# google/ffn

Hardware: NVIDIA H100
Metric: fov_steps_per_sec (higher is better)
Workload: dtype f16

## Files before the change

### ffn_b200/_lib.py

```python

from __future__ import annotations

import ctypes as C
import os

import numpy as np

HERE = os.path.dirname(os.path.abspath(__file__))
LIB_PATH = os.path.join(HERE, 'libffn_b200.so')

COMPUTE_FP16_TC = 0
COMPUTE_FP32 = 1
COMPUTE_FP16X2_TC = 2
IMAGE_U8 = 0
IMAGE_F32 = 1
ARRAY_SEED = 0
ARRAY_SEGMENTATION = 1
ARRAY_QPROB = 2
ARRAY_IMAGE = 3
MASK_MOVEMENT = 0
MASK_SEED = 1
SEED_POLICY_KINDS = {'peaks_2d': 0, 'fill_empty': 1, 'max_peaks': 2}

EXPORTS = [
    'ffn_last_error', 'ffn_engine_create', 'ffn_engine_destroy', 'ffn_engine_set_compute_mode', 'ffn_engine_set_chains', 'ffn_engine_set_grid',
    'ffn_engine_info', 'ffn_engine_profile', 'ffn_engine_trace', 'ffn_predict', 'ffn_canvas_create', 'ffn_canvas_destroy',
    'ffn_canvas_set_mask', 'ffn_canvas_segment_at', 'ffn_canvas_segment_all',
    'ffn_canvas_update_at', 'ffn_canvas_init_seed', 'ffn_canvas_read', 'ffn_canvas_write',
    'ffn_canvas_policy_state_size', 'ffn_canvas_policy_state_get', 'ffn_canvas_policy_state_set',
    'ffn_canvas_set_resume', 'ffn_canvas_trace', 'ffn_canvas_seed_peaks', 'ffn_canvas_seed_policy', 'ffn_canvas_set_max_id', 'ffn_canvas_get_counters', 'ffn_canvas_spec_stats', 'ffn_canvas_device_ptr',
    'ffn_canvas_add_id_offset', 'ffn_decision_points', 'ffn_reseg_eval', 'ffn_selftest_wgmma',
]


class ModelDesc(C.Structure):
  _fields_ = [('fov_zyx', C.c_int32 * 3), ('deltas_zyx', C.c_int32 * 3), ('depth', C.c_int32),
              ('features', C.c_int32)]


class Options(C.Structure):
  _fields_ = [('init_activation', C.c_float), ('pad_value', C.c_float),
# ... 71 lines not shown
  lib = C.CDLL(LIB_PATH)
  p = C.c_void_p
  i32p = C.POINTER(C.c_int32)
  lib.ffn_last_error.restype = C.c_char_p
  lib.ffn_last_error.argtypes = []
  lib.ffn_engine_create.argtypes = [C.c_int, C.POINTER(ModelDesc), C.POINTER(C.c_void_p),
                                    C.POINTER(C.c_void_p), C.c_int, C.POINTER(p)]
  lib.ffn_engine_destroy.argtypes = [p]
  lib.ffn_engine_destroy.restype = None
  lib.ffn_engine_set_compute_mode.argtypes = [p, C.c_int]
  lib.ffn_engine_set_grid.argtypes = [p, C.c_int]
  lib.ffn_engine_set_chains.argtypes = [p, C.c_int]
  lib.ffn_engine_info.argtypes = [p, C.POINTER(C.c_int64)]
  lib.ffn_engine_profile.argtypes = [p, C.POINTER(C.c_int64), C.c_int]
  lib.ffn_engine_trace.argtypes = [p, C.POINTER(C.c_int64), C.c_int64, C.c_int]
  lib.ffn_predict.argtypes = [p, p, p, C.c_int, p]
  lib.ffn_canvas_create.argtypes = [p, p, C.c_int, i32p, C.c_float, C.c_float, C.POINTER(Options),
                                    C.c_int, C.POINTER(p)]
  lib.ffn_canvas_destroy.argtypes = [p]
  lib.ffn_canvas_destroy.restype = None
  lib.ffn_canvas_set_mask.argtypes = [p, C.c_int, p]
  lib.ffn_canvas_segment_at.argtypes = [p, i32p, C.c_int, C.c_int64, C.POINTER(SegStats)]
  lib.ffn_canvas_segment_all.argtypes = [p, p, C.c_int64, p, C.c_int64, C.POINTER(C.c_int64), p,
                                         C.c_int64, C.POINTER(C.c_int64), C.POINTER(Counters)]
  lib.ffn_canvas_update_at.argtypes = [p, i32p, p]
  lib.ffn_canvas_init_seed.argtypes = [p, i32p]
  lib.ffn_canvas_read.argtypes = [p, C.c_int, i32p, i32p, p]
  lib.ffn_canvas_write.argtypes = [p, C.c_int, i32p, i32p, p]
  lib.ffn_canvas_policy_state_size.argtypes = [p, C.POINTER(C.c_int64), C.POINTER(C.c_int64)]
  lib.ffn_canvas_policy_state_get.argtypes = [p, p, p, i32p]
# ... 32 lines not shown
```

### ffn_b200/csrc/device_types.cuh

```cuda
#pragma once

#include <cuda.h>
#include <cuda_fp16.h>
#include <cuda_runtime.h>
#include <stdint.h>

#include "../../include/ffn_b200.h"

namespace ffn {

constexpr int kThreads = 320;
constexpr int kLoadWarp = 8;
constexpr int kSigWarp = 9;
constexpr int kActStages = 3;
constexpr int kTileM = 128;
constexpr int kTileOut = 126;
constexpr int kStackN = 96;
constexpr int kFeat = 32;
constexpr int kAccRegs = 64 * kStackN / 128;
constexpr int kMaxConv = 32;
constexpr int kMaxChains = 4;
constexpr int kBufsPerChain = 6;
constexpr int kMaxBufs = kMaxChains * kBufsPerChain;
constexpr int kSplitShift = 10;
// ... 13 lines not shown
  int rows_alloc;
  int V;
  float inv_pp, inv_xp;
};

struct Weights {
  const __half* w16;
  const __half* w16x2;
  const float* w32;
  const float* bias;
  const float* w_lom;
  float b_lom;
};

constexpr int kTraceEvents = 8, kTraceTiles = 2048, kTraceCta = 1;

constexpr unsigned kRowValid = 1, kRowX0 = 2, kRowXLast = 4;

struct Workspace {
  const uint8_t* row_flags;
  __half* act0_l;
  __half* act_l[2];
  float4* act0_f;
  float4* act_f[2];
  float4* res;
  unsigned* bar;
  int* abort_flag;
  long long* prof;
};

struct CanvasDev {
  const void* image;
  int image_is_u8;
  float mean, stddev;
  int* seg;
// ... 141 lines not shown
  Sched* sched;
  Ctl* ctl;
  unsigned* round_flag;
  CUtensorMap tmap[kMaxChains][3];
  int use_tmap;
  float* snap;
  Job job;
  int compute_mode;
};

constexpr int kStateSlot = 352;
constexpr int kOffMisc = 160;
constexpr int kMiscAbort = 7, kMiscDisco = 8, kMiscScratch = 16;
constexpr int kOffRound = kOffMisc + (kMiscScratch + 32 * kMaxChains) * 4;
constexpr int kOffProf = kOffRound + 2 * kMaxChains * 8 * 4;
constexpr int kOffXchg = (kOffProf + 16 * 8 + 15) / 16 * 16;
constexpr int kXchgBytes = 2 * 8 * 2 * 4 * 8 * 4;
constexpr int kBarsAreaBytes = kOffXchg + kXchgBytes;

struct SmemLayout {
  int wbuf;
  int act;
  int bias;
  int bars;
  int total;
};

__host__ __device__ inline SmemLayout smem_layout(const Geom& g) {
  SmemLayout s;
  s.wbuf = 0;
  s.act = 2 * 27 * 4 * 512;
// ... 10 lines not shown
  int x = 1;
  bool valid = false;
  if (m >= 1 && m <= kTileOut && r >= 0 && r < g.nr) {
    const int rem = r % g.pp, y = rem / g.xp;
    x = rem % g.xp;
    valid = y < g.fy;
  }
  return (valid ? kRowValid : 0u) | (x == 0 ? kRowX0 : 0u) | (x == g.fx - 1 ? kRowXLast : 0u);
}

inline uint8_t row_flags_byte(const Geom& g, int tile, int warp, int gq) {
  const int m0 = warp * 16 + gq;
  return (uint8_t)(row_flags_of(g, tile, m0) | row_flags_of(g, tile, m0 + 8) << 4);
}

__host__ __device__ inline size_t w16_layer_offset_halfs(int layer) {
  return layer == 0 ? 0 : (size_t)27 * 2 * 256 + (size_t)(layer - 1) * 27 * 4 * 256;
}
__host__ __device__ inline size_t w32_layer_offset_floats(int layer) {
  return layer == 0 ? 0 : (size_t)27 * 4 * 32 + (size_t)(layer - 1) * 27 * 32 * 32;
}

}
```

### ffn_b200/csrc/engine.cu

```cuda
#include <algorithm>
#include <cmath>
#include <cstdio>
#include <cstdlib>
#include <cstring>
#include <memory>
#include <string>
#include <vector>

#include "device_types.cuh"
#define FFN_KNS plain
#define FFN_PROFILE 0
#include "flood_kernel.cuh"
#undef FFN_KNS
#undef FFN_PROFILE
#define FFN_KNS profiled
#define FFN_PROFILE 1
#include "flood_kernel.cuh"
#undef FFN_KNS
#undef FFN_PROFILE
#include "seed_kernels.cuh"
#include "decision_kernels.cuh"
#include "reseg_kernels.cuh"
#include "selftest.cuh"

// ... 181 lines not shown
  p.round_flag = e->d_round_flag;
  p.snap = c ? c->d_snap : nullptr;
  std::memcpy(p.tmap, e->tmap, sizeof(p.tmap));
  p.use_tmap = e->use_tmap;
  p.job = job;
  {
    const char* env = std::getenv("FFN_B200_WATCHDOG_S");
    const long long secs = env ? std::atoll(env) : 60;
    p.job.watchdog_ns = (secs > 0 ? secs : 60) * 1000000000ll;
  }
  p.compute_mode = e->compute_mode;
  CUDA_OK(cudaMemsetAsync(e->ws.bar, 0, sizeof(unsigned), cudaStreamPerThread));
  CUDA_OK(cudaMemsetAsync(e->ws.abort_flag, 0, sizeof(int), cudaStreamPerThread));
  CUDA_OK(cudaMemsetAsync(e->d_ctl, 0, sizeof(Ctl), cudaStreamPerThread));
  CUDA_OK(cudaMemsetAsync(e->d_round_flag, 0, sizeof(unsigned), cudaStreamPerThread));
  for (int k = 0; k < kMaxChains; ++k) CUDA_OK(cudaMemsetAsync(e->cws[k].bar, 0, sizeof(unsigned), cudaStreamPerThread));
  void* args[] = {&p};
  CUDA_OK(cudaEventRecord(e->ev0, cudaStreamPerThread));
  CUDA_OK(cudaLaunchCooperativeKernel(flood_kernel(e), dim3(e->grid), dim3(kThreads), args, (size_t)e->smem_bytes,
                                      cudaStreamPerThread));
  CUDA_OK(cudaEventRecord(e->ev1, cudaStreamPerThread));
  CUDA_OK(cudaStreamSynchronize(cudaStreamPerThread));
  float ms = 0.f;
  CUDA_OK(cudaEventElapsedTime(&ms, e->ev0, e->ev1));
  e->last_kernel_seconds = ms * 1e-3;
  e->launches++;
  int abort_flag = 0;
  CUDA_OK(cudaMemcpy(&abort_flag, e->ws.abort_flag, sizeof(int), cudaMemcpyDeviceToHost));
  if (abort_flag != 0)
    return fail("device-side wait timed out (abort code " + std::to_string(abort_flag) +
// ... 216 lines not shown
  e->w.w_lom = d_wlom;
  e->w.b_lom = biases[g.nconv][0];
  e->owned = {d_w16, d_w16x2, d_w32, d_bias, d_wlom};

  Workspace& ws = e->ws;
  const size_t ra = (size_t)g.rows_alloc;
  if (dev_alloc(&ws.act0_l, 2 * ra * 8)) return 1;
  if (dev_alloc(&ws.act_l[0], 4 * ra * 8)) return 1;
  if (dev_alloc(&ws.act_l[1], 4 * ra * 8)) return 1;
  if (dev_alloc(&ws.act0_f, ra)) return 1;
  if (dev_alloc(&ws.act_f[0], 8 * ra)) return 1;
  if (dev_alloc(&ws.act_f[1], 8 * ra)) return 1;
  if (dev_alloc(&ws.res, 8 * ra)) return 1;
  if (dev_alloc(&ws.bar, 1)) return 1;
  if (dev_alloc(&ws.abort_flag, 1)) return 1;
  if (dev_alloc(&ws.prof, 32 + kTraceEvents * kTraceTiles)) return 1;
  for (void* p : std::vector<void*>{ws.act0_l, ws.act_l[0], ws.act_l[1], ws.act0_f, ws.act_f[0], ws.act_f[1], ws.res,
                                    ws.bar, ws.abort_flag, ws.prof})
    e->owned.push_back(p);
  {
    std::vector<uint8_t> flags((size_t)g.nt * 64);
    for (int t = 0; t < g.nt; ++t)
      for (int i = 0; i < 64; ++i) flags[(size_t)t * 64 + i] = row_flags_byte(g, t, i / 8, i % 8);
    uint8_t* d_flags = nullptr;
    if (dev_alloc(&d_flags, flags.size())) return 1;
    e->owned.push_back(d_flags);
    CUDA_OK(cudaMemcpy(d_flags, flags.data(), flags.size(), cudaMemcpyHostToDevice));
    ws.row_flags = d_flags;
  }
  for (int k = 0; k < kMaxChains; ++k) {
    ChainDev& cw = e->cws[k];
    if (dev_alloc(&cw.act0_h, 2 * ra * 8)) return 1;
    if (dev_alloc(&cw.act_h[0], 4 * ra * 8)) return 1;
    if (dev_alloc(&cw.act_h[1], 4 * ra * 8)) return 1;
    if (dev_alloc(&cw.seed_raw[0], (size_t)g.nt * kTileM)) return 1;
    if (dev_alloc(&cw.seed_raw[1], (size_t)g.nt * kTileM)) return 1;
    if (dev_alloc(&cw.logits, (size_t)g.nt * kTileM)) return 1;
    if (dev_alloc(&cw.count, 4)) return 1;
    if (dev_alloc(&cw.bar, 1)) return 1;
    if (dev_alloc(&cw.res, (size_t)g.nt * kTileM * kFeat)) return 1;
    for (void* p : std::vector<void*>{cw.act0_h, cw.act_h[0], cw.act_h[1], cw.seed_raw[0], cw.seed_raw[1], cw.logits,
                                      cw.count, cw.bar, cw.res})
      e->owned.push_back(p);
// ... 67 lines not shown
}

int ffn_engine_info(FfnEngine* e, int64_t info[8]) {
  if (!e || !info) return fail("null argument");
  info[0] = e->sm_count;
  info[1] = e->grid;
  info[2] = e->smem_bytes;
  info[3] = e->g.nt;
  info[4] = e->g.nr;
  info[5] = e->g.V;
  info[6] = e->launches;
  info[7] = (int64_t)(e->last_kernel_seconds * 1e9);
  return 0;
}

int ffn_engine_profile(FfnEngine* e, int64_t out[32], int reset) {
  if (!e) return fail("null argument");
  if (!out) {
    e->profiling = reset != 0;
    return 0;
  }
  if (set_device(e)) return 1;
  long long h[32];
  CUDA_OK(cudaMemcpy(h, e->ws.prof, sizeof(h), cudaMemcpyDeviceToHost));
  for (int i = 0; i < 32; ++i) out[i] = h[i];
  if (reset) CUDA_OK(cudaMemset(e->ws.prof, 0, sizeof(h)));
  return 0;
}

int ffn_engine_trace(FfnEngine* e, int64_t* out, int64_t n, int reset) {
  if (!e || !out || n < 0 || n > (int64_t)kTraceEvents * kTraceTiles) return fail("bad argument");
  if (set_device(e)) return 1;
  static_assert(sizeof(long long) == sizeof(int64_t), "trace element");
  CUDA_OK(cudaMemcpy(out, e->ws.prof + 32, (size_t)n * sizeof(int64_t), cudaMemcpyDeviceToHost));
  if (reset) CUDA_OK(cudaMemset(e->ws.prof + 32, 0, sizeof(long long) * kTraceEvents * kTraceTiles));
  return 0;
}

int ffn_predict(FfnEngine* e, const float* seed, const float* image, int batch, float* logits_out) {
  if (!e || !seed || !image || !logits_out || batch < 1) return fail("bad argument");
  if (set_device(e)) return 1;
  const size_t n = (size_t)batch * e->g.V;
  if (batch > e->predict_cap) {
    cudaFree(e->d_in_seed);
    cudaFree(e->d_in_image);
    cudaFree(e->d_out);
    e->d_in_seed = e->d_in_image = e->d_out = nullptr;
    if (dev_alloc(&e->d_in_seed, n, false)) return 1;
    if (dev_alloc(&e->d_in_image, n, false)) return 1;
    if (dev_alloc(&e->d_out, n, false)) return 1;
// ... 1079 lines not shown
```

### ffn_b200/csrc/flood_kernel.cuh

```cuda

#include <math_constants.h>

#include <utility>

#include "device_types.cuh"
#include "sm90.cuh"

namespace ffn {
namespace FFN_KNS {

struct Ctx {
  const KParams* p;
  int tid, warp, lane, cta, G;
  int t_begin, t_end;
  unsigned bar_target;
  unsigned ev0, ev1, ev2, ev3, ev4;
  unsigned round;
  unsigned long long t_start;
  unsigned char* smem;
  float* s_bias;
  uint64_t* mb_w;
  uint64_t* mb_full;
  uint64_t* mb_empty;
  uint64_t* mb_sig;
// ... 18 lines not shown
  return k == 0 ? c.ev0 : (k == 1 ? c.ev1 : (k == 2 ? c.ev2 : (k == 3 ? c.ev3 : c.ev4)));
}
__device__ __forceinline__ void ev_add(Ctx& c, int k, unsigned n) {
  if (k == 0) c.ev0 += n;
  else if (k == 1) c.ev1 += n;
  else if (k == 2) c.ev2 += n;
  else if (k == 3) c.ev3 += n;
  else c.ev4 += n;
}
__device__ __forceinline__ CanvasState* chain_state(const Ctx& c, int k) {
  return reinterpret_cast<CanvasState*>(reinterpret_cast<unsigned char*>(c.s_state) + k * kStateSlot);
}

__device__ __forceinline__ void chain_tiles(const Ctx& c, int k, int& tb, int& te) {
  const int nt = c.p->g.nt, base = nt / c.G, extra = nt % c.G;
  const int q = (c.cta + c.G - (k * extra) % c.G) % c.G;
  tb = q * base + min(q, extra);
  te = tb + base + (q < extra ? 1 : 0);
}

__device__ __forceinline__ bool aborted(const Ctx& c) {
  return sm90::ld_volatile_s32(c.p->ws.abort_flag) != 0;
}

#if FFN_PROFILE
__device__ __forceinline__ long long prof_now(const Ctx& c) { return c.prof ? clock64() : 0ll; }
__device__ __forceinline__ void prof_add(const Ctx& c, int slot, long long dt) {
  if (c.prof) c.prof[slot] += dt;
}
__device__ __forceinline__ void trace_ev(const Ctx& c, int ev, unsigned idx) {
  long long* trace = c.p->ws.prof;
  if (trace && c.cta == kTraceCta && idx < (unsigned)kTraceTiles) trace[32 + ev * kTraceTiles + idx] = clock64();
}
#else
__device__ __forceinline__ long long prof_now(const Ctx&) { return 0ll; }
__device__ __forceinline__ void prof_add(const Ctx&, int, long long) {}
__device__ __forceinline__ void trace_ev(const Ctx&, int, unsigned) {}
#endif

__device__ __forceinline__ void mbar_wait(const Ctx& c, uint64_t* bar, uint32_t parity) {
  unsigned spins = 0;
  long long t0 = 0;
  while (!sm90::mbar_try_wait(bar, parity)) {
    if ((++spins & 0x3FF) == 0) {
      if (aborted(c)) return;
      const long long now = clock64();
      if (t0 == 0) t0 = now;
// ... 397 lines not shown
  if (!(layer & 1)) return tc_epilogue<EPI_A, X2>(c, k, layer, tile, e, flags, d);
  if (layer == 1) return tc_epilogue<EPI_B_FIRST, X2>(c, k, layer, tile, e, flags, d);
  return tc_epilogue<EPI_B, X2>(c, k, layer, tile, e, flags, d);
}

__device__ __forceinline__ void publish_counts(Ctx& c, int k, int hit) {
  hit = __reduce_add_sync(0xffffffffu, hit);
  if (c.lane == 0 && hit) atomicAdd(&c.s_misc[k], hit);
  asm volatile("bar.sync 5, 256;" ::: "memory");
  if (c.tid == 0 && c.s_misc[k]) {
    const unsigned packed = (unsigned)c.s_misc[k];
    unsigned* cnt = c.p->ch[k].count + 2 * (c.round & 1u);
    if (packed & 0xffffu) atomicAdd(cnt, packed & 0xffffu);
    if (packed >> 16) atomicAdd(cnt + 1, packed >> 16);
  }
}

__device__ __forceinline__ void layers_pipelined(Ctx& c, unsigned mask) {
  const KParams& p = *c.p;
  const Geom& g = p.g;
  unsigned char* act_smem = c.smem + 2 * 27 * 4 * 512;
  const int seg_rows = kTileOut + 2 * g.halo;
  const int stage_bytes = 3 * 4 * seg_rows * 16;
  const int nconv = g.nconv;
  if (c.tid == 0) prof_add(c, 11, -prof_now(c));

  if (c.warp == kLoadWarp) {
    for (int layer = 0; layer < nconv; ++layer) {
      const int nch = layer == 0 ? 2 : 4;
      const unsigned n0 = c.load_cnt;
// ... 83 lines not shown
            tc_mma_issue<4>(d, a_lo, b_lo, seg_rows, g.xp, std::make_integer_sequence<int, 18>{});
          }
          const unsigned flags = tc_row_flags(c, tile);
          sm90::wgmma_wait_all();
          __syncwarp();
          if (c.lane == 0) sm90::mbar_arrive(&c.mb_empty[s]);
          if (c.tid == 0) prof_add(c, 3, prof_now(c) - t0);
          if (c.tid == 0) trace_ev(c, 4, c.epi_cnt);
          t0 = prof_now(c);
          hit += tc_epilogue_any<false>(c, k, layer, tile, e, flags, d);
          if (c.tid == 0) prof_add(c, 5, prof_now(c) - t0);
          if (c.tid == 0) trace_ev(c, 6, c.epi_cnt - 1u);
        }
        if (layer == nconv - 1) {
          publish_counts(c, k, hit);
        } else {
          chain_arrive_epi(c, k);
        }
      }
    }
  }
  bit_set(c, 8, true);
#pragma unroll
  for (int k = 0; k < kMaxChains; ++k)
    if ((mask >> k) & 1u) ev_add(c, k, (unsigned)nconv);
  if (c.tid == 0) prof_add(c, 11, prof_now(c));
}

__device__ __forceinline__ void tc_layer_x2(Ctx& c, int layer) {
  const KParams& p = *c.p;
// ... 120 lines not shown
  __syncthreads();
}

template <bool kSplit>
__device__ __forceinline__ void layers_blocking(Ctx& c) {
  const KParams& p = *c.p;
  grid_barrier(c);
  for (int layer = 0; layer < p.g.nconv; ++layer) {
    if constexpr (kSplit) {
      tc_layer_x2(c, layer);
    } else {
      f32_layer(c, layer);
    }
    if (layer + 1 < p.g.nconv) grid_barrier(c);
  }
}

__device__ __forceinline__ void tail_paste(Ctx& c, int k, int b, unsigned par, int pz, int py, int px, int batch_idx, bool disco) {
  const KParams& p = *c.p;
  const Geom& g = p.g;
  const ChainDev& ch = p.ch[k];
  const bool predict = p.job.mode == MODE_PREDICT;
  for (int r = c.t_begin * kTileOut + c.tid; r < c.t_end * kTileOut; r += kThreads) {
    int z, y, x;
    if (!row_to_zyx(g, r, z, y, x)) continue;
    const size_t fi = ((size_t)z * g.fy + y) * g.fx + x;
    if (predict) {
      p.job.out_logits[(size_t)batch_idx * g.V + fi] = __ldcg(ch.logits + r);
      continue;
    }
// ... 58 lines not shown
  CanvasState* st = L.st;
  if (st->q_tail >= p.cv.q_cap) {
    st->overflow |= 1;
    return;
  }
  const int t = st->q_tail++;
  trace_event(p, st, EV_PUSH, z, y, x);
  p.ob[L.b].q_score[t] = score;
  p.ob[L.b].q_pos[3 * t + 0] = z;
  p.ob[L.b].q_pos[3 * t + 1] = y;
  p.ob[L.b].q_pos[3 * t + 2] = x;
}

__device__ __forceinline__ int* policy_scratch(const Ctx& c, int k) { return c.s_misc + kMiscScratch + 32 * k; }

__device__ __forceinline__ void face_argmax(const Ctx& c, const LChain& L, int face) {
  const KParams& p = *c.p;
  const Geom& g = p.g;
  const ChainDev& ch = p.ch[L.k];
  int* scr = policy_scratch(c, L.k);
  float* s_score = reinterpret_cast<float*>(scr);
  int* s_rel = scr + 8;
  int* s_ok = scr + 26;
  const int cz = g.fz / 2, cy = g.fy / 2, cx = g.fx / 2;
  const int axis = face >> 1;
  const int dax = axis == 0 ? g.dz : (axis == 1 ? g.dy : g.dx);
  const int off = (face & 1) ? dax : -dax;
  const int d0 = axis == 0 ? g.dy : g.dz;
  const int d1 = axis == 2 ? g.dy : g.dx;
  const int n0 = 2 * d0 + 1, n1 = 2 * d1 + 1;
  const float* lgp = ch.logits;
  const float* odp = ch.seed_raw[L.par];
  int ok = 0;
  if (dax != 0) {
    float best = -CUDART_INF_F;
    int best_i = 0x7fffffff;
    constexpr int kPerLane = 10;
    for (int base = c.lane; base < n0 * n1; base += 32 * kPerLane) {
      float lg[kPerLane], od[kPerLane];
#pragma unroll
      for (int u = 0; u < kPerLane; ++u) {
        const int e = base + 32 * u;
        lg[u] = 0.f;
        od[u] = 0.f;
        if (e < n0 * n1) {
          const int i0 = e / n1, i1 = e - i0 * n1;
          const int z = axis == 0 ? cz + off : cz - g.dz + i0;
          const int y = axis == 0 ? cy - g.dy + i0 : (axis == 1 ? cy + off : cy - g.dy + i1);
          const int x = axis == 2 ? cx + off : cx - g.dx + i1;
          const int row = z * g.pp + y * g.xp + x;
          lg[u] = __ldcg(lgp + row);
          if (L.disco) od[u] = __ldcg(odp + row);
        }
      }
#pragma unroll
      for (int u = 0; u < kPerLane; ++u) {
        const int e = base + 32 * u;
        if (e < n0 * n1) {
          float v = lg[u];
          if (L.disco && od[u] < 0.f && v > od[u]) v = od[u];
          if (v > best || best_i == 0x7fffffff) {
            best = v;
            best_i = e;
          }
        }
      }
    }
#pragma unroll
    for (int s = 16; s > 0; s >>= 1) {
      const float ov = __shfl_xor_sync(0xffffffffu, best, s);
      const int oi = __shfl_xor_sync(0xffffffffu, best_i, s);
      if (oi != 0x7fffffff && (best_i == 0x7fffffff || ov > best || (ov == best && oi < best_i))) {
        best = ov;
        best_i = oi;
      }
    }
    if (c.lane == 0) {
      ok = (best >= p.cv.policy_th_f32) ? 1 : 0;
      const int i0 = best_i / n1, i1 = best_i - i0 * n1;
      const int r0 = i0 - n0 / 2, r1 = i1 - n1 / 2;
      s_score[face] = best;
      s_rel[3 * face + 0] = axis == 0 ? off : r0;
      s_rel[3 * face + 1] = axis == 0 ? r0 : (axis == 1 ? off : r1);
      s_rel[3 * face + 2] = axis == 2 ? off : r1;
    }
  }
  if (c.lane == 0) s_ok[face] = ok;
}

__device__ __forceinline__ void policy_finish(const Ctx& c, const LChain& L) {
  const KParams& p = *c.p;
  const ObjDev& ob = p.ob[L.b];
  CanvasState* st = L.st;
  int* scr = policy_scratch(c, L.k);
  const float* s_score = reinterpret_cast<const float*>(scr);
  const int* s_rel = scr + 8;
  const int* s_ok = scr + 26;
  const unsigned full = 0xffffffffu;
  const int f = c.lane;
  const bool mine = f < 6 && s_ok[f] != 0;
  const float sc = f < 6 ? s_score[f] : 0.f;
  const int rz = f < 6 ? s_rel[3 * f] : 0, ry = f < 6 ? s_rel[3 * f + 1] : 0, rx = f < 6 ? s_rel[3 * f + 2] : 0;
// ... 742 lines not shown
  if (c.tid == 0 && sm90::globaltimer_ns() - c.t_start > (unsigned long long)p.job.watchdog_ns) atomicExch(p.ws.abort_flag, 5);
  for (int i = c.tid; i < K * kStateWords; i += 256) {
    if (c.tid >= 256) break;
    const int k = i / kStateWords, w = i - k * kStateWords;
    const int b = __ldcg(&p.sched->active[k]);
    reinterpret_cast<unsigned long long*>(chain_state(c, k))[w] =
        __ldcg(reinterpret_cast<const unsigned long long*>(p.ob[b].st) + w);
  }
  if (c.tid >= 256)
    for (int i = c.tid - 256; i < kSchedWords; i += kThreads - 256)
      reinterpret_cast<unsigned long long*>(sc)[i] = __ldcg(reinterpret_cast<const unsigned long long*>(p.sched) + i);
  if (c.tid >= kThreads - kMaxChains) {
    const int k = c.tid - (kThreads - kMaxChains);
    if (k < K) c.s_misc[kMiscDisco + k] = (((stepped >> k) & 1u) && disco_active(p, k, par)) ? 1 : 0;
  }
  __syncthreads();
  const long long t_pol = prof_now(c);
  if (p.job.mode != MODE_UPDATE_AT) {
    for (int t = c.warp; t < K * 6; t += kThreads / 32) {
      const int k = t / 6, f = t - 6 * k;
      if (!((stepped >> k) & 1u)) continue;
      LChain L{k, sc->active[k], chain_state(c, k), par, c.s_misc[kMiscDisco + k] != 0};
      face_argmax(c, L, f);
    }
  }
  __syncthreads();
  if (c.warp < K && ((stepped >> c.warp) & 1u)) {
    LChain L{c.warp, sc->active[c.warp], chain_state(c, c.warp), par, c.s_misc[kMiscDisco + c.warp] != 0};
    if (L.st->phase == PH_AFTER_STEP) after_step(c, L);
  }
  if (c.tid == 0) prof_add(c, 12, prof_now(c) - t_pol);
  __syncthreads();
  if (c.warp == 0) {
    if (c.lane == 0) {
      sc->steps_executed += __popc(stepped);
    }
    __syncwarp();
    bool pause = false;
    if (p.job.step_budget > 0 && p.job.mode == MODE_SEGMENT) {
      const CanvasState* s0 = chain_state(c, 0);
      pause = s0->seg_all ? sc->steps_executed >= p.job.step_budget : s0->ctr.inference_calls >= p.job.step_budget;
    }
    int acts[kMaxChains];
    bool any = false;
#pragma unroll
    for (int k = 0; k < kMaxChains; ++k) {
      acts[k] = ACT_EXIT;
// ... 40 lines not shown
        if (!any) a = ACT_EXIT;
        else if (a == ACT_EXIT && k < K) a = ACT_IDLE;
        p.ctl->action[k] = k < K ? a : ACT_EXIT;
        if (k < K) {
          const CanvasState* s = chain_state(c, k);
          p.ctl->pos[k][0] = s->cur[0];
          p.ctl->pos[k][1] = s->cur[1];
          p.ctl->pos[k][2] = s->cur[2];
          p.ctl->buf[k] = sc->active[k];
        }
      }
    }
    __syncwarp();
  }
  __syncthreads();
  for (int i = c.tid; i < K * kStateWords; i += 256) {
    if (c.tid >= 256) break;
    const int k = i / kStateWords, w = i - k * kStateWords;
    reinterpret_cast<unsigned long long*>(p.ob[sc->active[k]].st)[w] = reinterpret_cast<const unsigned long long*>(chain_state(c, k))[w];
  }
  if (c.tid >= 256)
    for (int i = c.tid - 256; i < kSchedWords; i += kThreads - 256)
      reinterpret_cast<unsigned long long*>(p.sched)[i] = reinterpret_cast<const unsigned long long*>(sc)[i];
  __syncthreads();
  if (c.tid == 0) {
    sm90::red_release_add(p.round_flag, 1u);
    prof_add(c, 8, prof_now(c) - t_all);
  }
}

__device__ __forceinline__ void load3(const int* src, int (&dst)[3]) {
  dst[0] = __ldcg(src);
  dst[1] = __ldcg(src + 1);
  dst[2] = __ldcg(src + 2);
}

__device__ __forceinline__ void clear_dirty(Ctx& c, int b) {
  const KParams& p = *c.p;
  const CanvasState* st = p.ob[b].st;
  int dlo[3], dhi[3];
  load3(st->dirty_lo, dlo);
// ... 149 lines not shown
  c.mb_w = reinterpret_cast<uint64_t*>(smem_raw + L.bars);
  c.mb_full = c.mb_w + 2;
  c.mb_empty = c.mb_full + kActStages;
  c.mb_sig = c.mb_empty + kActStages;
  c.load_cnt = c.epi_cnt = 0;
  c.s_misc = reinterpret_cast<int*>(smem_raw + L.bars + kOffMisc);
  c.s_round = reinterpret_cast<int*>(smem_raw + L.bars + kOffRound);
  c.s_xchg = reinterpret_cast<float*>(smem_raw + L.bars + kOffXchg);
  c.s_state = reinterpret_cast<CanvasState*>(smem_raw + L.bars + kOffXchg);
  c.s_sched = reinterpret_cast<Sched*>(smem_raw + L.bars + kOffXchg + kMaxChains * kStateSlot);
  static_assert((2 + 2 * kActStages + kMaxChains) * 8 <= kOffMisc, "mbarrier area");
  static_assert(kMaxChains * kStateSlot + (int)sizeof(Sched) <= kXchgBytes, "leader working copies");
  c.prof = nullptr;
  if (FFN_PROFILE && p.ws.prof && (c.cta == 0 || c.cta == c.G - 1)) {
    c.prof = reinterpret_cast<long long*>(smem_raw + L.bars + kOffProf);
    if (c.tid < 16) c.prof[c.tid] = c.tid == 10 ? -clock64() : 0;
  }
#if FFN_PROFILE
  c.sig_cnt = 0;
#endif
  c.bits = 0;
  const bool tc = p.compute_mode != FFN_COMPUTE_FP32;
  const int K = p.nchains;

  for (int i = c.tid; i < p.g.nconv * 32; i += kThreads) c.s_bias[i] = p.w.bias[i];
  if (c.tid < 32) c.s_bias[p.g.nconv * 32 + c.tid] = p.w.w_lom[c.tid];
  if (c.tid == 0) c.s_bias[p.g.nconv * 32 + 32] = p.w.b_lom;
  if (c.tid < 2 * kMaxChains * 8) c.s_round[c.tid] = 0;
  if (tc) {
    if (c.tid == 0) {
      sm90::mbar_init(&c.mb_w[0], 1);
// ... 49 lines not shown
          const bool disco = disco_active(p, k, ppar);
          tail_paste(c, k, cur[4], ppar, cur[1], cur[2], cur[3], 0, disco);
          if (c.tid == 0) {
            prev[0] = 1 | (disco ? 2 : 0);
            prev[1] = cur[1];
            prev[2] = cur[2];
            prev[3] = cur[3];
            prev[4] = cur[4];
          }
        } else if (c.tid == 0) {
          prev[0] = 0;
        }
      }
      if (c.tid == 0) prof_add(c, 7, prof_now(c) - t_paste);
      if (c.tid == 0) {
        spin_until(c, p.round_flag, c.round + 1u, 4);
        c.s_misc[kMiscAbort] = sm90::ld_volatile_s32(p.ws.abort_flag);
      }
      __syncthreads();
      const int abort_now = c.s_misc[kMiscAbort];
      if (c.tid < K) {
        int* cur = c.s_round + 8 * c.tid;
        cur[0] = sm90::ld_volatile_s32(&p.ctl->action[c.tid]);
        cur[1] = sm90::ld_volatile_s32(&p.ctl->pos[c.tid][0]);
        cur[2] = sm90::ld_volatile_s32(&p.ctl->pos[c.tid][1]);
        cur[3] = sm90::ld_volatile_s32(&p.ctl->pos[c.tid][2]);
        cur[4] = sm90::ld_volatile_s32(&p.ctl->buf[c.tid]);
      }
      __syncthreads();
      if (abort_now != 0) break;
      bool all_exit = true;
// ... 17 lines not shown
          commit_write(c, b);
        }
      }
      if (c.tid == 0) prof_add(c, 6, prof_now(c) - t0);
      if (mask) {
        run_layers<kSplit>(c, mask);
        if (c.tid == 0) prof_add(c, 9, __popc(mask));
      }
      stepped = mask;
      ++c.round;
    }
  }

  if (c.tid == 0) prof_add(c, 10, prof_now(c));
  __syncthreads();
  if (c.prof && c.tid < 16) p.ws.prof[(c.cta == 0 ? 0 : 16) + c.tid] += c.prof[c.tid];
  if (tc && c.warp == 0 && bit_get(c, 8)) mbar_wait(c, &c.mb_w[0], bit_get(c, 0));
}

}

#ifndef FFN_MISC_KERNELS_DEFINED
#define FFN_MISC_KERNELS_DEFINED
__global__ void relabel_offset_kernel(int* seg, size_t n, int offset) {
  const size_t stride = (size_t)gridDim.x * blockDim.x;
  for (size_t i = (size_t)blockIdx.x * blockDim.x + threadIdx.x; i < n; i += stride) {
    const int v = seg[i];
    if (v > 0) seg[i] = v + offset;
  }
}

// ... 35 lines not shown
```

### ffn_b200/engine.py

```python

from __future__ import annotations

import ctypes as C
from typing import Optional, Sequence

import numpy as np
from scipy.special import logit

from . import _lib


def f32_logit(p: float) -> float:
  return float(np.float32(logit(float(np.float32(p)))))


def make_options(init_activation=0.95, pad_value=0.05, move_threshold=0.9, segment_threshold=0.6,
                 disco_seed_threshold=0.0, min_boundary_dist_zyx=(1, 1, 1), min_segment_size=1000,
                 policy_score_threshold: Optional[float] = None) -> _lib.Options:
  o = _lib.Options()
  o.init_activation = f32_logit(init_activation)
  o.pad_value = f32_logit(pad_value)
  o.move_threshold = f32_logit(move_threshold)
  o.segment_threshold = f32_logit(segment_threshold)
  o.disco_seed_threshold = float(np.float32(disco_seed_threshold))
# ... 58 lines not shown
  def set_chains(self, max_chains: int):
    _lib.check(self._lib.ffn_engine_set_chains(self._h, int(max_chains)))

  def set_compute_mode(self, mode: int):
    _lib.check(self._lib.ffn_engine_set_compute_mode(self._h, int(mode)))
    self.compute_mode = int(mode)

  def info(self) -> dict:
    buf = (C.c_int64 * 8)()
    _lib.check(self._lib.ffn_engine_info(self._h, buf))
    keys = ('sm_count', 'grid', 'smem_bytes', 'tiles', 'rows', 'fov_voxels', 'launches', 'last_kernel_ns')
    return dict(zip(keys, [int(v) for v in buf]))

  PROFILE_SLOTS = ('barrier_wait', 'act_tma_wait', 'weight_wait', 'mma', 'unused4', 'epi_body',
                   'stage', 'paste', 'leader', 'steps', 'kernel', 'conv_layers', 'leader_policy', 'leader_pops',
                   'chain_barrier_wait', 'unused')

  def enable_profiling(self, on: bool = True):
    _lib.check(self._lib.ffn_engine_profile(self._h, None, 1 if on else 0))

  def profile(self, reset: bool = True) -> dict:
    buf = (C.c_int64 * 32)()
    _lib.check(self._lib.ffn_engine_profile(self._h, buf, 1 if reset else 0))
    return {'cta0': dict(zip(self.PROFILE_SLOTS, [int(v) for v in buf[:16]])),
            'cta_last': dict(zip(self.PROFILE_SLOTS, [int(v) for v in buf[16:32]]))}

  def trace(self, reset: bool = True) -> np.ndarray:
    buf = np.zeros((8, 2048), dtype=np.int64)
    _lib.check(self._lib.ffn_engine_trace(self._h, buf.ctypes.data_as(C.POINTER(C.c_int64)), buf.size, 1 if reset else 0))
    return buf

  def predict(self, seed: np.ndarray, image: np.ndarray) -> np.ndarray:
    seed = np.ascontiguousarray(seed, dtype=np.float32)
    image = np.ascontiguousarray(image, dtype=np.float32)
    if seed.shape != image.shape:
      raise ValueError('seed and image shapes differ')
    single = seed.ndim == 3
    if seed.shape[-3:] != self.fov_zyx:
      raise ValueError('patch shape %r does not match the model FoV %r' % (seed.shape[-3:], self.fov_zyx))
    batch = 1 if single else seed.shape[0]
# ... 204 lines not shown
```

### include/ffn_b200.h

```cpp
#ifndef FFN_B200_H_
#define FFN_B200_H_

#include <stdint.h>

#ifdef __cplusplus
extern "C" {
#endif

typedef struct FfnEngine FfnEngine;
typedef struct FfnCanvas FfnCanvas;

enum {
  FFN_COMPUTE_FP16_TC = 0,
  FFN_COMPUTE_FP32 = 1,
  FFN_COMPUTE_FP16X2_TC = 2
};

enum { FFN_IMAGE_U8 = 0, FFN_IMAGE_F32 = 1 };

enum { FFN_ARRAY_SEED = 0, FFN_ARRAY_SEGMENTATION = 1, FFN_ARRAY_QPROB = 2, FFN_ARRAY_IMAGE = 3 };

enum { FFN_MASK_MOVEMENT = 0, FFN_MASK_SEED = 1 };

typedef struct {
// ... 54 lines not shown
  int64_t max_id;
  double device_seconds;
  int64_t kernel_launches;
} FfnCounters;

const char* ffn_last_error(void);

int ffn_engine_create(int device, const FfnModelDesc* model, const float* const* weights_dhwio,
                      const float* const* biases, int compute_mode, FfnEngine** out);
void ffn_engine_destroy(FfnEngine* engine);
int ffn_engine_set_compute_mode(FfnEngine* engine, int compute_mode);
int ffn_engine_set_chains(FfnEngine* engine, int max_chains);
int ffn_engine_set_grid(FfnEngine* engine, int num_ctas);
int ffn_engine_info(FfnEngine* engine, int64_t info[8]);

int ffn_engine_profile(FfnEngine* engine, int64_t out[32], int reset);
int ffn_engine_trace(FfnEngine* engine, int64_t* out, int64_t n, int reset);

int ffn_predict(FfnEngine* engine, const float* seed, const float* image, int batch,
                float* logits_out);

int ffn_canvas_create(FfnEngine* engine, const void* image, int image_dtype,
                      const int32_t shape_zyx[3], float image_mean, float image_stddev,
                      const FfnOptions* options, int keep_probability_maps, FfnCanvas** out);
void ffn_canvas_destroy(FfnCanvas* canvas);
int ffn_canvas_set_mask(FfnCanvas* canvas, int which, const uint8_t* mask);

int ffn_canvas_segment_at(FfnCanvas* canvas, const int32_t start_zyx[3], int reset,
                          int64_t max_steps, FfnSegStats* out);

int ffn_canvas_segment_all(FfnCanvas* canvas, const int32_t* seeds_zyx, int64_t n_seeds,
// ... 96 lines not shown
```

Baseline: 6353.

## Fuse face argmax into last conv layer epilogue via distributed atomic reduction

Moves the per-face argmax of the movement policy out of the single-CTA leader and into the last conv layer. Each CTA reduces the face voxels that fall in its own tiles, using a precomputed face table, and writes the result into global slots with packed 64-bit atomicMax keys. The leader then only unpacks six keys per chain instead of scanning face voxels serially. This is meant to shorten the serial leader phase between steps, at the cost of extra atomics and a table lookup in every CTA. The change also adds a spare-CTA offset to the chain tile assignment and widens the profiling slots.

```diff
diff --git a/ffn_b200/_lib.py b/ffn_b200/_lib.py
--- a/ffn_b200/_lib.py
+++ b/ffn_b200/_lib.py
@@ -24,7 +24,7 @@
 
 EXPORTS = [
     'ffn_last_error', 'ffn_engine_create', 'ffn_engine_destroy', 'ffn_engine_set_compute_mode', 'ffn_engine_set_chains', 'ffn_engine_set_grid',
-    'ffn_engine_info', 'ffn_engine_profile', 'ffn_engine_trace', 'ffn_predict', 'ffn_canvas_create', 'ffn_canvas_destroy',
+    'ffn_engine_info', 'ffn_engine_profile', 'ffn_engine_trace', 'ffn_face_table', 'ffn_predict', 'ffn_canvas_create', 'ffn_canvas_destroy',
     'ffn_canvas_set_mask', 'ffn_canvas_segment_at', 'ffn_canvas_segment_all',
     'ffn_canvas_update_at', 'ffn_canvas_init_seed', 'ffn_canvas_read', 'ffn_canvas_write',
     'ffn_canvas_policy_state_size', 'ffn_canvas_policy_state_get', 'ffn_canvas_policy_state_set',
@@ -126,6 +126,8 @@
   lib.ffn_engine_info.argtypes = [p, C.POINTER(C.c_int64)]
   lib.ffn_engine_profile.argtypes = [p, C.POINTER(C.c_int64), C.c_int]
   lib.ffn_engine_trace.argtypes = [p, C.POINTER(C.c_int64), C.c_int64, C.c_int]
+  lib.ffn_face_table.argtypes = [C.POINTER(ModelDesc), C.c_int64, C.POINTER(C.c_int32), C.POINTER(C.c_int64),
+                                 C.POINTER(C.c_int32), C.POINTER(C.c_int64)]
   lib.ffn_predict.argtypes = [p, p, p, C.c_int, p]
   lib.ffn_canvas_create.argtypes = [p, p, C.c_int, i32p, C.c_float, C.c_float, C.POINTER(Options),
                                     C.c_int, C.POINTER(p)]
diff --git a/ffn_b200/csrc/device_types.cuh b/ffn_b200/csrc/device_types.cuh
--- a/ffn_b200/csrc/device_types.cuh
+++ b/ffn_b200/csrc/device_types.cuh
@@ -4,6 +4,10 @@
 #include <cuda_fp16.h>
 #include <cuda_runtime.h>
 #include <stdint.h>
+#include <string.h>
+
+#include <algorithm>
+#include <vector>
 
 #include "../../include/ffn_b200.h"
 
@@ -51,11 +55,21 @@
 };
 
 constexpr int kTraceEvents = 8, kTraceTiles = 2048, kTraceCta = 1;
+constexpr int kProfSlots = 32;
 
 constexpr unsigned kRowValid = 1, kRowX0 = 2, kRowXLast = 4;
+
+struct alignas(8) FaceEntry {
+  int row;
+  int face_e;
+};
+constexpr int kFaceSlots = 12;
 
 struct Workspace {
   const uint8_t* row_flags;
+  const FaceEntry* face_tab;
+  const int* face_first;
+  unsigned long long* face_best;
   __half* act0_l;
   __half* act_l[2];
   float4* act0_f;
@@ -227,7 +241,7 @@
 constexpr int kMiscAbort = 7, kMiscDisco = 8, kMiscScratch = 16;
 constexpr int kOffRound = kOffMisc + (kMiscScratch + 32 * kMaxChains) * 4;
 constexpr int kOffProf = kOffRound + 2 * kMaxChains * 8 * 4;
-constexpr int kOffXchg = (kOffProf + 16 * 8 + 15) / 16 * 16;
+constexpr int kOffXchg = (kOffProf + kProfSlots * 8 + 15) / 16 * 16;
 constexpr int kXchgBytes = 2 * 8 * 2 * 4 * 8 * 4;
 constexpr int kBarsAreaBytes = kOffXchg + kXchgBytes;
 
@@ -268,6 +282,43 @@
   return (uint8_t)(row_flags_of(g, tile, m0) | row_flags_of(g, tile, m0 + 8) << 4);
 }
 
+inline void build_face_table(const Geom& g, std::vector<FaceEntry>& tab, std::vector<int>& first) {
+  const int c[3] = {g.fz / 2, g.fy / 2, g.fx / 2}, d[3] = {g.dz, g.dy, g.dx};
+  tab.clear();
+  for (int face = 0; face < 6; ++face) {
+    const int axis = face >> 1, a0 = axis == 0 ? 1 : 0, a1 = axis == 2 ? 1 : 2;
+    if (d[axis] == 0) continue;
+    const int n1 = 2 * d[a1] + 1;
+    for (int e = 0; e < (2 * d[a0] + 1) * n1; ++e) {
+      int zyx[3];
+      zyx[axis] = c[axis] + ((face & 1) ? d[axis] : -d[axis]);
+      zyx[a0] = c[a0] - d[a0] + e / n1;
+      zyx[a1] = c[a1] - d[a1] + e % n1;
+      tab.push_back({zyx[0] * g.pp + zyx[1] * g.xp + zyx[2], face << 24 | e});
+    }
+  }
+  std::stable_sort(tab.begin(), tab.end(), [](const FaceEntry& a, const FaceEntry& b) { return a.row < b.row; });
+  first.assign((size_t)g.nt + 1, 0);
+  for (int t = 0, i = 0; t <= g.nt; ++t) {
+    while (i < (int)tab.size() && tab[i].row < t * kTileOut) ++i;
+    first[t] = i;
+  }
+}
+
+__host__ __device__ inline unsigned long long face_key(float score, int e) {
+  if (score == 0.f) score = 0.f;
+  unsigned b;
+  memcpy(&b, &score, 4);
+  b ^= (b >> 31) ? 0xffffffffu : 0x80000000u;
+  return (unsigned long long)b << 32 | (0xffffffffu - (unsigned)e);
+}
+__host__ __device__ inline void face_key_unpack(unsigned long long key, float& score, int& e) {
+  unsigned b = (unsigned)(key >> 32);
+  b ^= (b >> 31) ? 0x80000000u : 0xffffffffu;
+  memcpy(&score, &b, 4);
+  e = (int)(0xffffffffu - (unsigned)key);
+}
+
 __host__ __device__ inline size_t w16_layer_offset_halfs(int layer) {
   return layer == 0 ? 0 : (size_t)27 * 2 * 256 + (size_t)(layer - 1) * 27 * 4 * 256;
 }
diff --git a/ffn_b200/csrc/engine.cu b/ffn_b200/csrc/engine.cu
--- a/ffn_b200/csrc/engine.cu
+++ b/ffn_b200/csrc/engine.cu
@@ -219,6 +219,7 @@
   CUDA_OK(cudaMemsetAsync(e->ws.abort_flag, 0, sizeof(int), cudaStreamPerThread));
   CUDA_OK(cudaMemsetAsync(e->d_ctl, 0, sizeof(Ctl), cudaStreamPerThread));
   CUDA_OK(cudaMemsetAsync(e->d_round_flag, 0, sizeof(unsigned), cudaStreamPerThread));
+  CUDA_OK(cudaMemsetAsync(e->ws.face_best, 0, sizeof(unsigned long long) * kMaxChains * kFaceSlots, cudaStreamPerThread));
   for (int k = 0; k < kMaxChains; ++k) CUDA_OK(cudaMemsetAsync(e->cws[k].bar, 0, sizeof(unsigned), cudaStreamPerThread));
   void* args[] = {&p};
   CUDA_OK(cudaEventRecord(e->ev0, cudaStreamPerThread));
@@ -465,7 +466,7 @@
   if (dev_alloc(&ws.res, 8 * ra)) return 1;
   if (dev_alloc(&ws.bar, 1)) return 1;
   if (dev_alloc(&ws.abort_flag, 1)) return 1;
-  if (dev_alloc(&ws.prof, 32 + kTraceEvents * kTraceTiles)) return 1;
+  if (dev_alloc(&ws.prof, 2 * kProfSlots + kTraceEvents * kTraceTiles)) return 1;
   for (void* p : std::vector<void*>{ws.act0_l, ws.act_l[0], ws.act_l[1], ws.act0_f, ws.act_f[0], ws.act_f[1], ws.res,
                                     ws.bar, ws.abort_flag, ws.prof})
     e->owned.push_back(p);
@@ -478,6 +479,21 @@
     e->owned.push_back(d_flags);
     CUDA_OK(cudaMemcpy(d_flags, flags.data(), flags.size(), cudaMemcpyHostToDevice));
     ws.row_flags = d_flags;
+  }
+  {
+    std::vector<FaceEntry> tab;
+    std::vector<int> first;
+    build_face_table(g, tab, first);
+    FaceEntry* d_tab = nullptr;
+    int* d_first = nullptr;
+    if (dev_alloc(&d_tab, std::max<size_t>(tab.size(), 1))) return 1;
+    if (dev_alloc(&d_first, first.size())) return 1;
+    if (dev_alloc(&ws.face_best, (size_t)kMaxChains * kFaceSlots)) return 1;
+    for (void* p : std::vector<void*>{d_tab, d_first, ws.face_best}) e->owned.push_back(p);
+    CUDA_OK(cudaMemcpy(d_tab, tab.data(), tab.size() * sizeof(FaceEntry), cudaMemcpyHostToDevice));
+    CUDA_OK(cudaMemcpy(d_first, first.data(), first.size() * sizeof(int), cudaMemcpyHostToDevice));
+    ws.face_tab = d_tab;
+    ws.face_first = d_first;
   }
   for (int k = 0; k < kMaxChains; ++k) {
     ChainDev& cw = e->cws[k];
@@ -575,17 +591,36 @@
   return 0;
 }
 
-int ffn_engine_profile(FfnEngine* e, int64_t out[32], int reset) {
+int ffn_engine_profile(FfnEngine* e, int64_t out[64], int reset) {
   if (!e) return fail("null argument");
   if (!out) {
     e->profiling = reset != 0;
     return 0;
   }
   if (set_device(e)) return 1;
-  long long h[32];
+  static_assert(2 * kProfSlots == 64, "ffn_engine_profile's out[64]");
+  long long h[2 * kProfSlots];
   CUDA_OK(cudaMemcpy(h, e->ws.prof, sizeof(h), cudaMemcpyDeviceToHost));
-  for (int i = 0; i < 32; ++i) out[i] = h[i];
+  for (int i = 0; i < 2 * kProfSlots; ++i) out[i] = h[i];
   if (reset) CUDA_OK(cudaMemset(e->ws.prof, 0, sizeof(h)));
+  return 0;
+}
+
+int ffn_face_table(const FfnModelDesc* model, int64_t cap, int32_t* entries, int64_t* n_entries, int32_t* tile_first,
+                   int64_t* n_tiles) {
+  if (!model || !n_entries || !n_tiles) return fail("null argument");
+  const Geom g = make_geom(*model);
+  std::vector<FaceEntry> tab;
+  std::vector<int> first;
+  build_face_table(g, tab, first);
+  *n_entries = (int64_t)tab.size();
+  *n_tiles = g.nt;
+  for (size_t i = 0; entries && i < tab.size() && (int64_t)i < cap; ++i) {
+    entries[3 * i] = tab[i].row;
+    entries[3 * i + 1] = tab[i].face_e >> 24;
+    entries[3 * i + 2] = tab[i].face_e & 0xffffff;
+  }
+  if (tile_first) std::copy(first.begin(), first.end(), tile_first);
   return 0;
 }
 
@@ -593,8 +628,8 @@
   if (!e || !out || n < 0 || n > (int64_t)kTraceEvents * kTraceTiles) return fail("bad argument");
   if (set_device(e)) return 1;
   static_assert(sizeof(long long) == sizeof(int64_t), "trace element");
-  CUDA_OK(cudaMemcpy(out, e->ws.prof + 32, (size_t)n * sizeof(int64_t), cudaMemcpyDeviceToHost));
-  if (reset) CUDA_OK(cudaMemset(e->ws.prof + 32, 0, sizeof(long long) * kTraceEvents * kTraceTiles));
+  CUDA_OK(cudaMemcpy(out, e->ws.prof + 2 * kProfSlots, (size_t)n * sizeof(int64_t), cudaMemcpyDeviceToHost));
+  if (reset) CUDA_OK(cudaMemset(e->ws.prof + 2 * kProfSlots, 0, sizeof(long long) * kTraceEvents * kTraceTiles));
   return 0;
 }
 
diff --git a/ffn_b200/csrc/flood_kernel.cuh b/ffn_b200/csrc/flood_kernel.cuh
--- a/ffn_b200/csrc/flood_kernel.cuh
+++ b/ffn_b200/csrc/flood_kernel.cuh
@@ -56,7 +56,8 @@
 
 __device__ __forceinline__ void chain_tiles(const Ctx& c, int k, int& tb, int& te) {
   const int nt = c.p->g.nt, base = nt / c.G, extra = nt % c.G;
-  const int q = (c.cta + c.G - (k * extra) % c.G) % c.G;
+  const int spare = (c.p->job.mode != MODE_PREDICT && c.p->nchains * extra <= c.G - 1) ? 1 : 0;
+  const int q = (c.cta + c.G - (spare + k * extra) % c.G) % c.G;
   tb = q * base + min(q, extra);
   te = tb + base + (q < extra ? 1 : 0);
 }
@@ -72,7 +73,7 @@
 }
 __device__ __forceinline__ void trace_ev(const Ctx& c, int ev, unsigned idx) {
   long long* trace = c.p->ws.prof;
-  if (trace && c.cta == kTraceCta && idx < (unsigned)kTraceTiles) trace[32 + ev * kTraceTiles + idx] = clock64();
+  if (trace && c.cta == kTraceCta && idx < (unsigned)kTraceTiles) trace[2 * kProfSlots + ev * kTraceTiles + idx] = clock64();
 }
 #else
 __device__ __forceinline__ long long prof_now(const Ctx&) { return 0ll; }
@@ -500,6 +501,45 @@
     if (packed & 0xffffu) atomicAdd(cnt, packed & 0xffffu);
     if (packed >> 16) atomicAdd(cnt + 1, packed >> 16);
   }
+}
+
+__device__ __forceinline__ void face_reduce(const Ctx& c, int k, int tb, int te, int nwarps) {
+  const KParams& p = *c.p;
+  const int e0 = __ldg(p.ws.face_first + tb), e1 = __ldg(p.ws.face_first + te);
+  if (e0 == e1) return;
+  const long long t0 = prof_now(c);
+  const ChainDev& ch = p.ch[k];
+  const bool both = p.cv.opt.disco_seed_threshold >= 0.f;
+  unsigned long long* slots = p.ws.face_best + k * kFaceSlots;
+  for (int base = e0 + 32 * c.warp; base < e1; base += 32 * nwarps) {
+    const int i = base + c.lane;
+    const bool have = i < e1;
+    int face = 0;
+    unsigned long long key = 0, key_d = 0;
+    if (have) {
+      const int2 en = __ldg(reinterpret_cast<const int2*>(p.ws.face_tab + i));
+      face = en.y >> 24;
+      const float v = __ldcg(ch.logits + en.x);
+      key = face_key(v, en.y & 0xffffff);
+      if (both) {
+        const float o = __ldcg(ch.seed_raw[c.round & 1u] + en.x);
+        key_d = face_key((o < 0.f && v > o) ? o : v, en.y & 0xffffff);
+      }
+    }
+    unsigned faces = __reduce_or_sync(0xffffffffu, have ? 1u << face : 0u);
+    while (faces) {
+      const int f = __ffs(faces) - 1;
+      faces &= faces - 1;
+      const bool mine = have && face == f;
+      for (int variant = 0; variant < (both ? 2 : 1); ++variant) {
+        const unsigned long long mk = mine ? (variant ? key_d : key) : 0ull;
+        const unsigned hi = __reduce_max_sync(0xffffffffu, (unsigned)(mk >> 32));
+        const unsigned lo = __reduce_max_sync(0xffffffffu, (unsigned)(mk >> 32) == hi ? (unsigned)mk : 0u);
+        if (c.lane == 0) atomicMax(slots + 6 * variant + f, (unsigned long long)hi << 32 | lo);
+      }
+    }
+  }
+  if (c.tid == 0) prof_add(c, 20, prof_now(c) - t0);
 }
 
 __device__ __forceinline__ void layers_pipelined(Ctx& c, unsigned mask) {
@@ -613,6 +653,10 @@
         }
         if (layer == nconv - 1) {
           publish_counts(c, k, hit);
+          if (p.job.mode == MODE_SEGMENT) {
+            chain_tiles(c, k, tb, te);
+            face_reduce(c, k, tb, te, 8);
+          }
         } else {
           chain_arrive_epi(c, k);
         }
@@ -763,6 +807,10 @@
     }
     if (layer + 1 < p.g.nconv) grid_barrier(c);
   }
+  if (p.job.mode == MODE_SEGMENT) {
+    __syncthreads();
+    face_reduce(c, 0, c.t_begin, c.t_end, kThreads / 32);
+  }
 }
 
 __device__ __forceinline__ void tail_paste(Ctx& c, int k, int b, unsigned par, int pz, int py, int px, int batch_idx, bool disco) {
@@ -851,78 +899,37 @@
 
 __device__ __forceinline__ int* policy_scratch(const Ctx& c, int k) { return c.s_misc + kMiscScratch + 32 * k; }
 
-__device__ __forceinline__ void face_argmax(const Ctx& c, const LChain& L, int face) {
+__device__ __forceinline__ void face_pick(const Ctx& c, int k, int face, bool disco) {
   const KParams& p = *c.p;
   const Geom& g = p.g;
-  const ChainDev& ch = p.ch[L.k];
-  int* scr = policy_scratch(c, L.k);
+  int* scr = policy_scratch(c, k);
   float* s_score = reinterpret_cast<float*>(scr);
   int* s_rel = scr + 8;
   int* s_ok = scr + 26;
-  const int cz = g.fz / 2, cy = g.fy / 2, cx = g.fx / 2;
+  unsigned long long* slots = p.ws.face_best + k * kFaceSlots;
+  const unsigned long long key = __ldcg(slots + (disco ? 6 : 0) + face);
+  slots[face] = 0ull;
+  slots[6 + face] = 0ull;
   const int axis = face >> 1;
   const int dax = axis == 0 ? g.dz : (axis == 1 ? g.dy : g.dx);
   const int off = (face & 1) ? dax : -dax;
   const int d0 = axis == 0 ? g.dy : g.dz;
   const int d1 = axis == 2 ? g.dy : g.dx;
   const int n0 = 2 * d0 + 1, n1 = 2 * d1 + 1;
-  const float* lgp = ch.logits;
-  const float* odp = ch.seed_raw[L.par];
   int ok = 0;
   if (dax != 0) {
-    float best = -CUDART_INF_F;
-    int best_i = 0x7fffffff;
-    constexpr int kPerLane = 10;
-    for (int base = c.lane; base < n0 * n1; base += 32 * kPerLane) {
-      float lg[kPerLane], od[kPerLane];
-#pragma unroll
-      for (int u = 0; u < kPerLane; ++u) {
-        const int e = base + 32 * u;
-        lg[u] = 0.f;
-        od[u] = 0.f;
-        if (e < n0 * n1) {
-          const int i0 = e / n1, i1 = e - i0 * n1;
-          const int z = axis == 0 ? cz + off : cz - g.dz + i0;
-          const int y = axis == 0 ? cy - g.dy + i0 : (axis == 1 ? cy + off : cy - g.dy + i1);
-          const int x = axis == 2 ? cx + off : cx - g.dx + i1;
-          const int row = z * g.pp + y * g.xp + x;
-          lg[u] = __ldcg(lgp + row);
-          if (L.disco) od[u] = __ldcg(odp + row);
-        }
-      }
-#pragma unroll
-      for (int u = 0; u < kPerLane; ++u) {
-        const int e = base + 32 * u;
-        if (e < n0 * n1) {
-          float v = lg[u];
-          if (L.disco && od[u] < 0.f && v > od[u]) v = od[u];
-          if (v > best || best_i == 0x7fffffff) {
-            best = v;
-            best_i = e;
-          }
-        }
-      }
-    }
-#pragma unroll
-    for (int s = 16; s > 0; s >>= 1) {
-      const float ov = __shfl_xor_sync(0xffffffffu, best, s);
-      const int oi = __shfl_xor_sync(0xffffffffu, best_i, s);
-      if (oi != 0x7fffffff && (best_i == 0x7fffffff || ov > best || (ov == best && oi < best_i))) {
-        best = ov;
-        best_i = oi;
-      }
-    }
-    if (c.lane == 0) {
-      ok = (best >= p.cv.policy_th_f32) ? 1 : 0;
-      const int i0 = best_i / n1, i1 = best_i - i0 * n1;
-      const int r0 = i0 - n0 / 2, r1 = i1 - n1 / 2;
-      s_score[face] = best;
-      s_rel[3 * face + 0] = axis == 0 ? off : r0;
-      s_rel[3 * face + 1] = axis == 0 ? r0 : (axis == 1 ? off : r1);
-      s_rel[3 * face + 2] = axis == 2 ? off : r1;
-    }
-  }
-  if (c.lane == 0) s_ok[face] = ok;
+    float best;
+    int best_i;
+    face_key_unpack(key, best, best_i);
+    ok = (best >= p.cv.policy_th_f32) ? 1 : 0;
+    const int i0 = best_i / n1, i1 = best_i - i0 * n1;
+    const int r0 = i0 - n0 / 2, r1 = i1 - n1 / 2;
+    s_score[face] = best;
+    s_rel[3 * face + 0] = axis == 0 ? off : r0;
+    s_rel[3 * face + 1] = axis == 0 ? r0 : (axis == 1 ? off : r1);
+    s_rel[3 * face + 2] = axis == 2 ? off : r1;
+  }
+  s_ok[face] = ok;
 }
 
 __device__ __forceinline__ void policy_finish(const Ctx& c, const LChain& L) {
@@ -1695,23 +1702,20 @@
     const int k = c.tid - (kThreads - kMaxChains);
     if (k < K) c.s_misc[kMiscDisco + k] = (((stepped >> k) & 1u) && disco_active(p, k, par)) ? 1 : 0;
   }
+  if (p.job.mode == MODE_SEGMENT && c.tid < K * 6) {
+    const int k = c.tid / 6;
+    if ((stepped >> k) & 1u) face_pick(c, k, c.tid - 6 * k, disco_active(p, k, par));
+  }
   __syncthreads();
   const long long t_pol = prof_now(c);
-  if (p.job.mode != MODE_UPDATE_AT) {
-    for (int t = c.warp; t < K * 6; t += kThreads / 32) {
-      const int k = t / 6, f = t - 6 * k;
-      if (!((stepped >> k) & 1u)) continue;
-      LChain L{k, sc->active[k], chain_state(c, k), par, c.s_misc[kMiscDisco + k] != 0};
-      face_argmax(c, L, f);
-    }
-  }
-  __syncthreads();
+  if (c.tid == 0) prof_add(c, 16, t_pol - t_all);
   if (c.warp < K && ((stepped >> c.warp) & 1u)) {
     LChain L{c.warp, sc->active[c.warp], chain_state(c, c.warp), par, c.s_misc[kMiscDisco + c.warp] != 0};
     if (L.st->phase == PH_AFTER_STEP) after_step(c, L);
   }
-  if (c.tid == 0) prof_add(c, 12, prof_now(c) - t_pol);
   __syncthreads();
+  const long long t_adv = prof_now(c);
+  if (c.tid == 0) prof_add(c, 12, t_adv - t_pol);
   if (c.warp == 0) {
     if (c.lane == 0) {
       sc->steps_executed += __popc(stepped);
@@ -1782,6 +1786,8 @@
     __syncwarp();
   }
   __syncthreads();
+  const long long t_out = prof_now(c);
+  if (c.tid == 0) prof_add(c, 17, t_out - t_adv);
   for (int i = c.tid; i < K * kStateWords; i += 256) {
     if (c.tid >= 256) break;
     const int k = i / kStateWords, w = i - k * kStateWords;
@@ -1793,6 +1799,7 @@
   __syncthreads();
   if (c.tid == 0) {
     sm90::red_release_add(p.round_flag, 1u);
+    prof_add(c, 18, prof_now(c) - t_out);
     prof_add(c, 8, prof_now(c) - t_all);
   }
 }
@@ -1972,7 +1979,7 @@
   c.prof = nullptr;
   if (FFN_PROFILE && p.ws.prof && (c.cta == 0 || c.cta == c.G - 1)) {
     c.prof = reinterpret_cast<long long*>(smem_raw + L.bars + kOffProf);
-    if (c.tid < 16) c.prof[c.tid] = c.tid == 10 ? -clock64() : 0;
+    if (c.tid < kProfSlots) c.prof[c.tid] = c.tid == 10 ? -clock64() : 0;
   }
 #if FFN_PROFILE
   c.sig_cnt = 0;
@@ -2052,7 +2059,9 @@
       }
       if (c.tid == 0) prof_add(c, 7, prof_now(c) - t_paste);
       if (c.tid == 0) {
+        const long long t_flag = prof_now(c);
         spin_until(c, p.round_flag, c.round + 1u, 4);
+        prof_add(c, 19, prof_now(c) - t_flag);
         c.s_misc[kMiscAbort] = sm90::ld_volatile_s32(p.ws.abort_flag);
       }
       __syncthreads();
@@ -2100,7 +2109,7 @@
 
   if (c.tid == 0) prof_add(c, 10, prof_now(c));
   __syncthreads();
-  if (c.prof && c.tid < 16) p.ws.prof[(c.cta == 0 ? 0 : 16) + c.tid] += c.prof[c.tid];
+  if (c.prof && c.tid < kProfSlots) p.ws.prof[(c.cta == 0 ? 0 : kProfSlots) + c.tid] += c.prof[c.tid];
   if (tc && c.warp == 0 && bit_get(c, 8)) mbar_wait(c, &c.mb_w[0], bit_get(c, 0));
 }
 
diff --git a/ffn_b200/engine.py b/ffn_b200/engine.py
--- a/ffn_b200/engine.py
+++ b/ffn_b200/engine.py
@@ -96,16 +96,18 @@
 
   PROFILE_SLOTS = ('barrier_wait', 'act_tma_wait', 'weight_wait', 'mma', 'unused4', 'epi_body',
                    'stage', 'paste', 'leader', 'steps', 'kernel', 'conv_layers', 'leader_policy', 'leader_pops',
-                   'chain_barrier_wait', 'unused')
+                   'chain_barrier_wait', 'unused', 'leader_copy_in', 'leader_advance', 'leader_copy_out',
+                   'round_flag_wait', 'face_reduce') + ('unused',) * 11
 
   def enable_profiling(self, on: bool = True):
     _lib.check(self._lib.ffn_engine_profile(self._h, None, 1 if on else 0))
 
   def profile(self, reset: bool = True) -> dict:
-    buf = (C.c_int64 * 32)()
+    n = len(self.PROFILE_SLOTS)
+    buf = (C.c_int64 * (2 * n))()
     _lib.check(self._lib.ffn_engine_profile(self._h, buf, 1 if reset else 0))
-    return {'cta0': dict(zip(self.PROFILE_SLOTS, [int(v) for v in buf[:16]])),
-            'cta_last': dict(zip(self.PROFILE_SLOTS, [int(v) for v in buf[16:32]]))}
+    return {'cta0': dict(zip(self.PROFILE_SLOTS, [int(v) for v in buf[:n]])),
+            'cta_last': dict(zip(self.PROFILE_SLOTS, [int(v) for v in buf[n:]]))}
 
   def trace(self, reset: bool = True) -> np.ndarray:
     buf = np.zeros((8, 2048), dtype=np.int64)
diff --git a/include/ffn_b200.h b/include/ffn_b200.h
--- a/include/ffn_b200.h
+++ b/include/ffn_b200.h
@@ -92,7 +92,9 @@
 int ffn_engine_set_grid(FfnEngine* engine, int num_ctas);
 int ffn_engine_info(FfnEngine* engine, int64_t info[8]);
 
-int ffn_engine_profile(FfnEngine* engine, int64_t out[32], int reset);
+int ffn_engine_profile(FfnEngine* engine, int64_t out[64], int reset);
+int ffn_face_table(const FfnModelDesc* model, int64_t cap, int32_t* entries, int64_t* n_entries, int32_t* tile_first,
+                   int64_t* n_tiles);
 int ffn_engine_trace(FfnEngine* engine, int64_t* out, int64_t n, int reset);
 
 int ffn_predict(FfnEngine* engine, const float* seed, const float* image, int batch,
```

New measurement: 6548, median of 6. 1.03x the previous value.
